# pangsu0613/TransCAR

Hardware: AMD Instinct MI355X
Metric: nuScenes frames/sec (6-cam+radar, 900 queries): fusion decoder (Detr3DHead.forward + box decode), FPN features resident in HBM (higher is better)
Workload: dtype f32 (linear steps and attention core of the batched launches: f16x2 split operands, 3 v_mfma_f32_16x16x32_f16 products, fp32 accumulate; activations of the 32-row tiles held as two f16 planes; 4- / 8-row tiles: f32 MFMA)

## Files before the change

transcar_amd/csrc/chain.hip:

```cpp
#include <stdlib.h>
#include <string.h>

#include <type_traits>

#include "kernels.hpp"
#ifdef TC_CHAIN_STAMPS
__device__ long long g_cam_stamps[4][8];
#define CAM_STAMP(slot)                                                                        \
  do {                                                                                         \
    if (blockIdx.x == 100 && (threadIdx.x & 63) == 0)                                          \
      g_cam_stamps[(threadIdx.x >> 6) & 3][(slot)] = __builtin_amdgcn_s_memtime();             \
  } while (0)
#endif
#include "rowdev.hpp"
#define TC_ONCE_LD(p) ldg4_stream(p)
#ifdef TC_CHAIN_DUMP
__device__ float* g_chain_dump;
__device__ long long g_chain_dump_floats;
#endif

namespace tc {

namespace {

constexpr int CH_NW = 4;
constexpr int CH_NT = CH_NW * 64;
constexpr int CH_NW_MAX = 8;
constexpr int nw_of(int R) { return R == 32 ? 8 : 4; }
constexpr int LD5 = 516;
constexpr int LD2 = 260;
constexpr int LDL = 36;

struct StepRes {
  const float* p0; const float* p1; const float* p2; const float* p3;
  float* gd; float* gt;
  int K, N, gld, gmod;
  short kind, src, src2, dst, res, act, flags, sync, rep, si;
  int src_off, src2_off;
  int pad_;
};
struct EpiRec {
  float* gd; float* gt;
  int dst_off, res_off, dst_ld, res_ld;
  int gld, act, flags, N;
  int has_bias, woff;
  int drop_site;
  int pad1;
};
struct PreRec { const float* first; int nidx; int pad; };
template <int NW> struct StepAllT { StepRes r; EpiRec e; PreRec p[NW]; };
using StepAll = StepAllT<CH_NW>;
static_assert(sizeof(StepAllT<CH_NW>) % 16 == 0 && sizeof(StepAllT<CH_NW_MAX>) % 16 == 0, "records are copied 16 bytes at a time");
template <int N, int NW = CH_NW> struct Recs { StepAllT<NW> s[N]; };

constexpr int HM_WORDS = 8;
static_assert(HM_WORDS * 8 <= LDL * 4 && (LDL * 4) % 8 == 0, "hit masks live in a row of the logit buffer");
template <int R, int NREC>
struct ChainLds {
  StepAllT<nw_of(R)> recs[NREC];
  float unit[4][R][LD2];
  float l[R][LDL];
  float box[R][12];
  float cen[R][4];
  int gate[R];
  int rowg[R];
};
static_assert(LD5 * 1 <= 2 * LD2, "the 512-wide tile must fit two units");

#ifdef TC_CHAIN_STAMPS
#define CHAIN_DBG(v) (v)
#else
#define CHAIN_DBG(v) 0
#endif

#define MFMA44(a, b, c, grp) __builtin_amdgcn_mfma_f32_4x4x1f32((a), (b), (c), 4, (grp), 0)

enum Buf : short { B_NONE = -1, B_A = 0 , B_X , B_U1, B_U2, B_U3, B_L };
enum Kind : short {
  K_END = 0, K_LOAD, K_LINEAR, K_LN, K_POSENC, K_SAMPLE, K_REFUPD, K_TOKENS, K_RADAR_ATTN, K_BOXADD, K_RADAR_GATE,
  K_NARROW,
  K_NOP,
  K_LOADG,
  K_MASKCOPY,
  K_LN_BWD,
  K_ATTN_BWD,
  K_BOXSIG
};
enum NSpecial : short { N_LOGITS = -1, N_CODE = -2, N_CLS = -3 };
// ... 171 lines not shown
enum TSel : short { T_NONE = -1, T_QP = 0, T_AO, T_X1, T_X2, T_H, T_FF, T_X3, T_C0, T_C1, T_C2, T_C3, T_T0, T_T1, T_TREG,
                    E_U0, E_U1, E_U2, E_POS, E_F0, E_F1, E_F2, E_MEM, T_COUNT };
constexpr short RADAR_TAPE[17] = {T_NONE, T_QP, T_AO, T_X1, T_X2, T_H, T_FF, T_X3, T_C0, T_T0, T_C1, T_T1, T_C2, T_C3,
                                  T_TREG, T_NONE, T_NONE};
constexpr short ENC_TAPE[10] = {T_NONE, E_U1, E_F0, E_U2, E_F1, E_F2, E_MEM, T_NONE, T_NONE, T_NONE};
constexpr short ENC_TAPE2[10] = {T_NONE, E_U0, T_NONE, T_NONE, T_NONE, T_NONE, E_POS, T_NONE, T_NONE, T_NONE};
constexpr short BWD_TAPE[19] = {T_NONE, T_T1, T_T0, T_NONE, T_NONE, T_NONE, T_C2, T_NONE, T_C0, T_NONE, T_X2, T_NONE,
                                T_H, T_NONE, T_X1, T_NONE, T_NONE, T_NONE, T_NONE};
constexpr short BWD_TAPE2[19] = {T_NONE, T_NONE, T_NONE, T_NONE, T_NONE, T_NONE, T_C3, T_NONE, T_C1, T_NONE, T_FF, T_NONE,
                                 T_NONE, T_NONE, T_NONE, T_NONE, T_NONE, T_NONE, T_NONE};

constexpr int MAX_PAIRS = 48;
constexpr int RADAR_PAIRS = 14;

struct ChainDev {
  int program, M, Q, code, ncls, nlogits, has_next, nlayers;
  int total, early_n;
  float* g[G_COUNT]; int g_ld[G_COUNT]; int g_mod[G_COUNT];
  float qscale; int qpad;
  DropK drop;
  int dbg;
  int tile_rows;
  int matrix_path;
  int last_cls_only;
  const float* ref_in; int ref_mod; float* ref_out; float* box_m;
  CamK cam; unsigned long long* pair_counter;
  const float* pre; const int* premask;
  const float* tokens; int RI, T, pad_mult;
  const float* ref_last; const float* box_in;
  int cen_from_box;
  float rmin[TC_MAX_RADAR_LAYERS], rmax[TC_MAX_RADAR_LAYERS];
  float* all_box; int* hits;
  const int* row_perm;
  float* tape[T_COUNT]; size_t tape_stride; size_t hits_stride;
  DropK rdrop;
  const float* bwd_cxy[TC_MAX_RADAR_LAYERS]; int bwd_ldc[TC_MAX_RADAR_LAYERS];
  const float* bwd_box[TC_MAX_RADAR_LAYERS];
  int* range_status;
  const float* loss_vals;
  float* loss_out;
  const DetAcc* detp;
};
struct ChainK : ChainDev {
  tc_linear pairs[MAX_PAIRS];
  tc_linear gpairs[MAX_PAIRS];
  float* dy[D_COUNT]; size_t dy_stride = 0;
  const float* d_cls = nullptr; const float* d_box = nullptr;
  float* dkv[TC_MAX_RADAR_LAYERS] = {nullptr, nullptr, nullptr};
  size_t w16_delta = 0;
  int npoints = 1;
  int refine = 1;
  int l0_seq = 0;
};

inline bool generic_xattn(const ChainK& k) { return k.npoints > 1 || k.cam.num_levels < 4; }

constexpr int table_steps(int prog) {
  return (prog == PROG_DECODER ? (int)(sizeof(PROG_DECODER_T) / sizeof(StepDesc))
          : prog == PROG_PROLOGUE ? (int)(sizeof(PROG_PROLOGUE_T) / sizeof(StepDesc))
          : prog_is_enc_full(prog) ? (int)(sizeof(PROG_RADAR_ENC_T) / sizeof(StepDesc))
          : prog == PROG_RADAR_ENC_A ? (int)(sizeof(PROG_RADAR_ENC_A_T) / sizeof(StepDesc))
          : prog == PROG_RADAR_ENC_B ? (int)(sizeof(PROG_RADAR_ENC_B_T) / sizeof(StepDesc))
          : prog == PROG_RADAR_BWD ? (int)(sizeof(PROG_RADAR_BWD_T) / sizeof(StepDesc))
          : prog == PROG_DECODER_HEADS ? (int)(sizeof(PROG_DECODER_HEADS_T) / sizeof(StepDesc))
                                     : (int)(sizeof(PROG_RADAR_LAYER_T) / sizeof(StepDesc))) - 1;
}
// ... 1078 lines not shown
#pragma unroll
        for (int ri = 0; ri < EARLY_RW; ++ri) {
          int grow = min(m0 + wave + ri * NW, M - 1);
          if (mod > 0) grow = grow % mod;
          early_v[j][ri] = TC_ONCE_LD(gsrc + (size_t)grow * ld + 4 * lane);
        }
      }
    }
    START_STAMP(41);
#pragma unroll
    for (int j = 0; j < EARLY_MAX; ++j) {
      if (j < early_n) {
        float* dst = reinterpret_cast<float*>(smem_raw) + recs[j].e.dst_off;
#pragma unroll
        for (int ri = 0; ri < EARLY_RW; ++ri) {
          const int row = wave + ri * NW;
          if (row < R) act_st4<PL>(dst + row * LD2, 4 * lane, early_v[j][ri]);
        }
      }
    }
  }
#pragma unroll
  for (int t = 0; t < REC_TRIPS; ++t) {
    const int i = threadIdx.x + t * NT;
    if (i < REC16) reinterpret_cast<int4*>(&S.recs[0])[i] = rec_v[t];
  }
  START_STAMP(43);

  if (prog_is_radar(PROG)) {
    auto row_of = [&](int row) {
      const int pos = min(m0 + row, M - 1);
      return k.row_perm != nullptr ? k.row_perm[pos] : pos;
    };
    if (threadIdx.x < R) S.rowg[threadIdx.x] = row_of(threadIdx.x);
    for (int row = wave; row < R; row += NW) {
      const int grow = row_of(row);
      act_st4<PL>(&S.unit[0][row][0], 4 * lane, TC_ONCE_LD(k.g[G_QF] + (size_t)grow * 256 + 4 * lane));
    }
    {
      const int row = threadIdx.x >> 4, j = threadIdx.x & 15;
      if (row < R) {
        const int grow = row_of(row);
        if (j < k.code) S.box[row][j] = k.box_in[(size_t)grow * k.code + j];
        if (j >= 12 && j < 15) {
          const int c = j - 12;
          if (k.cen_from_box) {
            S.cen[row][c] = k.box_in[(size_t)grow * k.code + (c == 2 ? 4 : c)];
          } else {
            const float r = k.ref_last[(size_t)grow * 3 + c];
            const float* pc = k.cam.pc;
            S.cen[row][c] = c < 2 ? __fadd_rn(__fmul_rn(r, pc[3 + c] - pc[c]), pc[c]) : r;
          }
        }
      }
    }
  }
  if constexpr (PROG == PROG_RADAR_BWD) {
    for (int i = threadIdx.x; i < R * LD2; i += NT) (&S.unit[0][0][0])[i] = 0.0f;
    if (threadIdx.x < R * 12) (&S.box[0][0])[threadIdx.x] = 0.0f;
    if (threadIdx.x < R) S.gate[threadIdx.x] = 0;
  }
  __syncthreads();

  START_STAMP(46);
#ifdef TC_CHAIN_STAMPS
  int stamp_i = 0;
  STEP_STAMP();
#endif

  auto do_ln = [&](const StepRes& r) {
    constexpr int NR = R / NW;
    const float* a = buf_ptr(S, r.src); const int lda = buf_ld(r.src);
    const float* c = buf_ptr(S, r.src2); const int ldc = buf_ld(r.src2);
    const bool xp = (r.flags & F_LN_XP) != 0;
    const float* dd = xp ? nullptr : buf_ptr(S, r.res);
// ... 51 lines not shown
    s.dst = nullptr; s.dst_ld = 0; s.res = nullptr; s.res_ld = 0; s.gate = nullptr;
    s.act = 0; s.scale = 1.0f; s.scale_cols = 0;
    s.gdst = nullptr; s.gdst_ld = 0; s.gt = nullptr; s.gt_ld = 0; s.gt_rpb = 1;
    s.m0 = m0; s.M = M;
    s.woff = (r.flags & F_WAVE1) ? 1 : 0;
    s.dbg = k.dbg;
    s.sub_on = 0;
    s.drop_site = 0; s.drop_seed = 0; s.drop_thr = 0; s.drop_scale = 1.0f; s.drop_stride = 0; s.drop_q = 0;
    s.rowg = nullptr; s.gpre = 0; s.cmask = nullptr; s.cscale = 1.0f;
    s.dst_pl = 0; s.res_pl = 0; s.range_flag = nullptr;
    return s;
  };
  auto epi_spec = [&](int j) {
    const EpiRec e = load_uniform<EpiRec>(S.recs[j].e);
    float* base = reinterpret_cast<float*>(smem_raw);
    LinSpec s;
    s.K = 0; s.N = e.N; s.W = nullptr;
    s.bias = e.has_bias ? base : nullptr;
    s.src = nullptr; s.src_ld = 0; s.src2 = nullptr; s.src2_ld = 0;
    s.dst = e.dst_off >= 0 ? base + e.dst_off : nullptr; s.dst_ld = e.dst_ld;
    s.res = e.res_off >= 0 ? base + e.res_off : nullptr; s.res_ld = e.res_ld;
    s.gate = (e.flags & F_GATE) ? &S.gate[0] : nullptr;
    s.act = e.act;
    s.scale = (e.flags & F_SCALEQ) ? k.qscale : 1.0f; s.scale_cols = (e.flags & F_SCALEQ) ? 256 : 0;
    s.gdst = e.gd; s.gdst_ld = e.gld;
    s.gt = (e.flags & F_CMASK) ? nullptr : e.gt; s.gt_ld = k.qpad; s.gt_rpb = k.Q;
    s.cmask = (e.flags & F_CMASK) ? e.gt : nullptr;
    s.cscale = (e.flags & F_CMASK_SCALE) ? k.rdrop.scale : 1.0f;
    s.m0 = m0; s.M = M;
    s.woff = e.woff;
    s.dbg = 0;
    s.sub_on = 0;
    s.drop_site = 0; s.drop_seed = 0; s.drop_thr = 0; s.drop_scale = 1.0f; s.drop_stride = 0; s.drop_q = 0;
    s.rowg = (prog_is_radar(PROG) && k.row_perm != nullptr) ? &S.rowg[0] : nullptr;
    s.gpre = (e.flags & F_GPRE) ? 1 : 0;
    s.dst_pl = PL && e.dst_ld != LDL; s.res_pl = PL && e.res_ld != LDL;
    s.range_flag = MM == 1 ? k.range_status : nullptr;
    if (DROP) {
      if constexpr (PROG == PROG_RADAR_TRAIN) {
        s.drop_site = e.drop_site; s.drop_seed = k.rdrop.seed; s.drop_thr = k.rdrop.thr; s.drop_scale = k.rdrop.scale;
      } else {
        s.drop_site = e.drop_site; s.drop_seed = k.drop.seed; s.drop_thr = k.drop.thr; s.drop_scale = k.drop.scale;
        s.drop_stride = k.drop.seed_stride; s.drop_q = (int)k.drop.rows_per_sample;
      }
    }
    return s;
  };

  auto tile_has_hit = [&]() {
    int any = 0;
#pragma unroll
    for (int i = 0; i < R; ++i) any |= S.gate[i];
    return __builtin_amdgcn_readfirstlane(any) > 0;
  };

#ifdef TC_CHAIN_DUMP
  auto dump_step = [&](int step, int dst_id) {
    if constexpr (PROG == PROG_RADAR) {
      __syncthreads();
      float* out = g_chain_dump;
      const float* src = buf_ptr(S, dst_id);
      if (out != nullptr && src != nullptr && dst_id != B_L && (long long)(step + 1) * M * 256 <= g_chain_dump_floats) {
        const int ld = buf_ld(dst_id);
        for (int row = wave; row < R; row += NW)
          if (m0 + row < M)
            st4(out + ((size_t)step * M + S.rowg[row]) * 256 + 4 * lane, *reinterpret_cast<const float4*>(src + row * ld + 4 * lane));
      }
// ... 1146 lines not shown

template <bool MP>
static int launch_dual(const ChainK& kd, const ChainK& ke, int part, hipStream_t s) {
  const int rows = tile_rows(kd);
  const char* what = "chain(decoder + radar_encode)";
#define TC_DUAL(RA, RB, MM, PRE)                                                                      \
  (part == 1 ? launch_dual_r<RA, RB, PROG_RADAR_ENC_A, MM, PRE, MP>(kd, ke, s, what)                  \
   : part == 2 ? launch_dual_r<RA, RB, PROG_RADAR_ENC_B, MM, PRE, MP>(kd, ke, s, what)                \
               : launch_dual_r<RA, RB, PROG_RADAR_ENC, MM, PRE, MP>(kd, ke, s, what))
  if (rows == 4) return TC_DUAL(4, 4, 0, false);
  if (rows == 8) return TC_DUAL(8, 8, 0, false);
  if (rows == 32) {
    TC_REQUIRE(use_f16x2(kd), "%s: 32-row tiles exist on the f16x2 matrix path only", what);
    if (kd.pre != nullptr) return TC_DUAL(32, 32, 1, true);
    return TC_DUAL(32, 32, 1, false);
  }
  if (use_f16x2(kd) && kd.pre != nullptr) return TC_DUAL(16, 16, 1, true);
  if (use_f16x2(kd)) return TC_DUAL(16, 16, 1, false);
  return TC_DUAL(16, 16, 0, false);
#undef TC_DUAL
}

int launch_decoder_chain_with_encoders(const DecoderChainArgs& d, const RadarEncodeArgs& e, int part,
                                       hipStream_t s) {
  ChainK kd, ke;
  int rc = make_decoder_k(d, kd);
  if (rc != 0) return rc;
  rc = make_radar_enc_k(e, ke, part);
  if (rc != 0) return rc;
  TC_REQUIRE(kd.drop.thr == 0, "decoder dropout: launch the encoders on their own (launch_radar_encode)");
  return generic_xattn(kd) ? launch_dual<true>(kd, ke, part, s) : launch_dual<false>(kd, ke, part, s);
}

int launch_radar_chain(const RadarChainArgs& a, hipStream_t s) {
  TC_REQUIRE(a.code <= 10 && a.ncls <= 32, "radar_chain: code=%d ncls=%d", a.code, a.ncls);
  TC_REQUIRE(a.nlayers >= 1 && a.nlayers <= TC_MAX_RADAR_LAYERS, "radar_chain: nlayers=%d", a.nlayers);
  ChainK k;
  init_k(k);
  k.program = PROG_RADAR; k.M = a.M; k.Q = a.Q; k.code = a.code; k.ncls = a.ncls; k.nlayers = a.nlayers;
  k.w16_delta = a.w[0].packed16_delta;
  k.row_perm = a.row_perm;
  k.has_next = 1;
  for (int r = 0; r < a.nlayers; ++r) {
    const tc_radar_layer& w = a.w[r];
    tc_linear* p = &k.pairs[r * RADAR_PAIRS];
    p[0] = w.attn.in_proj; p[1] = w.attn.out_proj; p[2] = tc_linear{w.norm2.g, w.norm2.b};
    p[3] = w.linear1; p[4] = w.linear2; p[5] = tc_linear{w.norm3.g, w.norm3.b};
    p[6] = w.final_cls.l0; p[7] = tc_linear{w.final_cls.n1.g, w.final_cls.n1.b}; p[8] = w.final_cls.l3;
    p[9] = tc_linear{w.final_cls.n4.g, w.final_cls.n4.b}; p[10] = w.final_cls.l6;
    p[11] = w.final_reg.l0; p[12] = w.final_reg.l2; p[13] = w.final_reg.l4;
    k.rmin[r] = w.radius_min; k.rmax[r] = w.radius_max;
    k.g[G_KV0 + r] = const_cast<float*>(a.kv[r]);
  }
  k.g[G_QF] = const_cast<float*>(a.qf);
  k.g[G_CLS] = a.all_cls; k.g_ld[G_CLS] = a.ncls;
  k.qscale = a.qscale;
  k.tokens = a.tokens; k.RI = a.RI; k.T = a.T; k.pad_mult = a.pad_mult;
  k.ref_last = a.ref_last; k.box_in = a.box_m; k.cen_from_box = a.cen_from_box;
  TC_REQUIRE(a.cen_from_box || a.ref_last != nullptr, "radar_chain: ref_last is null");
  for (int i = 0; i < 6; ++i) k.cam.pc[i] = a.pc[i];
  k.all_box = a.all_box; k.hits = a.hits;
  TC_REQUIRE(a.tile_rows == 0 || a.tile_rows == 4 || a.tile_rows == 8 || a.tile_rows == 16 || a.tile_rows == 32,
             "radar_chain: tile_rows=%d (0 = automatic, 4, 8, 16 or 32)", a.tile_rows);
  k.tile_rows = a.tile_rows; k.last_cls_only = a.last_cls_only; k.matrix_path = a.matrix_path;
  k.range_status = a.range_status;
  if (a.tape != nullptr) {
    TC_REQUIRE(a.row_perm == nullptr && !a.last_cls_only, "radar_chain: the training forward takes the rows in their own order");
    k.program = PROG_RADAR_TRAIN;
    for (int i = 0; i < T_COUNT; ++i) k.tape[i] = a.tape[i];
    k.tape_stride = a.tape_stride; k.hits_stride = a.hits_stride; k.rdrop = a.drop;
    if (k.tile_rows >= 16 || (k.tile_rows == 0 && a.M > 2048)) k.tile_rows = 8;
  }
  return launch(k, s, "chain(radar)");
}
// ... 155 lines not shown
```

transcar_amd/csrc/head.hip:

```cpp
#include <math.h>
#include <stdarg.h>
#include <stdlib.h>
#include <string.h>

#include "kernels.hpp"

namespace tc {

static thread_local char g_err[512] = "";

void set_error(const char* fmt, ...) {
  va_list ap;
  va_start(ap, fmt);
  vsnprintf(g_err, sizeof(g_err), fmt, ap);
  va_end(ap);
}

int check_launch(const char* what) {
  hipError_t e = hipGetLastError();
  if (e != hipSuccess) {
    set_error("%s: %s", what, hipGetErrorString(e));
    return (int)e;
  }
  return 0;
// ... 253 lines not shown
      }
    }
    if (radar && !ddrop && lid == enc_first) TC_TRY(launch_decoder_chain_with_encoders(d, re, L > 1 ? 1 : 0, s));
    else if (radar && !ddrop && L > 1 && lid == enc_first + 1) TC_TRY(launch_decoder_chain_with_encoders(d, re, 2, s));
    else TC_TRY(launch_decoder_chain(d, s));
  }
  if (opt.phase == 1) return 0;
  if (!refine)
    TC_TRY(launch_ref_broadcast(folded ? w->l0_init_reference : h.init_ref, folded ? Q : 0, h.inter_refs, rows, L, s));
  if (aux) {
    if (aux->init_reference) {
      if (folded) {
        for (int b = 0; b < B; ++b)
          TC_HIP(hipMemcpyAsync(aux->init_reference + (size_t)b * Q * 3, w->l0_init_reference,
                                (size_t)Q * 3 * 4, hipMemcpyDeviceToDevice, s));
      } else {
        TC_HIP(hipMemcpyAsync(aux->init_reference, h.init_ref, (size_t)rows * 3 * 4, hipMemcpyDeviceToDevice, s));
      }
    }
  }
  if (!radar) return 0;
  RadarChainArgs rc;
  rc.qf = h.hs + (size_t)(L - 1) * rows * C;
  rc.ref_last = h.inter_refs + (size_t)(L - 1) * rows * 3;
  rc.box_m = h.box_m; rc.tokens = radar_tokens; rc.RI = w->radar_in_dims;
  for (int r = 0; r < TC_MAX_RADAR_LAYERS; ++r) { rc.kv[r] = h.kv3[r]; rc.w[r] = w->radar[r]; }
  rc.nlayers = w->num_radar_layers; rc.Q = Q; rc.T = T; rc.pad_mult = pad_mult; rc.code = code;
  rc.ncls = ncls; rc.M = rows; rc.qscale = 1.0f / sqrtf((float)(C / TC_RADAR_HEADS));
  for (int i = 0; i < 6; ++i) rc.pc[i] = w->pc_range[i];
  rc.all_cls = all_cls_scores; rc.all_box = all_bbox_preds; rc.hits = h.hits;
  rc.tile_rows = opt.chain_tile_rows; rc.last_cls_only = opt.last_level_cls_only; rc.matrix_path = opt.matrix_path;
  rc.range_status = opt.range_status;
  if (opt.radar_row_order == 2 || (opt.radar_row_order == 0 && rows > 1024)) {
    TC_TRY(launch_radar_compact(rc.ref_last, rc.box_m, code, 0, w->pc_range, radar_tokens, w->radar_in_dims, B, Q, T,
                                w->radar[0].radius_min, w->radar[0].radius_max, h.hitflag, h.perm, s));
    rc.row_perm = h.perm;
  }
  TC_TRY(launch_radar_chain(rc, s));
  if (aux && aux->radar_hit_counts)
    TC_HIP(hipMemcpyAsync(aux->radar_hit_counts, h.hits, (size_t)w->num_radar_layers * rows * 4,
                          hipMemcpyDeviceToDevice, s));
  return 0;
}

struct PackItem { const float* src; int N, K; const float** slot; bool narrow; bool absent; };

static int collect_pack_items(const tc_head_weights* w, tc_head_weights* v, PackItem* it) {
  const int C = w->embed_dims, F = w->ffn_dims, NL = w->num_cams * w->num_levels * head_points(w);
  const int code = w->code_size, ncls = w->num_classes;
  int n = 0;
  auto add = [&](const tc_linear& src, tc_linear& dst, int N, int K, bool narrow = false, bool absent = false) {
    it[n].src = src.w; it[n].N = N; it[n].K = K; it[n].slot = &dst.w; it[n].narrow = narrow; it[n].absent = absent; ++n;
  };
  add(w->reference_points, v->reference_points, 3, C);
  for (int l = 0; l < w->num_layers; ++l) {
    const tc_decoder_layer& a = w->layers[l]; tc_decoder_layer& b = v->layers[l];
    add(a.self_attn.in_proj, b.self_attn.in_proj, 3 * C, C);
    add(a.self_attn.out_proj, b.self_attn.out_proj, C, C);
    add(a.attention_weights, b.attention_weights, NL, C);
    add(a.output_proj, b.output_proj, C, C);
    add(a.position_encoder.l3, b.position_encoder.l3, C, C);
    add(a.ffn0, b.ffn0, F, C);
    add(a.ffn1, b.ffn1, C, F);
    const bool noreg = a.reg.l0.w == nullptr;
    add(a.reg.l0, b.reg.l0, C, C, false, noreg);
    add(a.reg.l2, b.reg.l2, C, C, false, noreg);
    add(a.reg.l4, b.reg.l4, code, C, true, noreg);
  }
  if (w->num_radar_layers > 0) {
// ... 306 lines not shown
  TC_TRY(read_options(options, opt));
  HeadWs h;
  const size_t need = head_ws_layout(w, B, T, workspace, workspace_bytes, &h);
  TC_REQUIRE(need <= workspace_bytes, "workspace too small: need %zu, have %zu", need, workspace_bytes);
  hipStream_t s = as_stream(stream);
  const int Q = w->num_query, C = w->embed_dims, rows = B * Q, rt = B * T;
  const int code = w->code_size, ncls = w->num_classes;
  RadarEncodeArgs re;
  re.tokens = radar_tokens; re.RI = w->radar_in_dims; re.M = rt;
  re.rpe = w->radar_position_encoder; re.f0 = w->radar_feat0; re.f2 = w->radar_feat2;
  re.f4 = w->radar_feat4; re.nlayers = w->num_radar_layers;
  for (int r = 0; r < TC_MAX_RADAR_LAYERS; ++r) {
    const tc_mha& m = w->radar[r].attn;
    re.kvproj[r] = tc_linear{m.in_proj.w ? m.in_proj.w + (size_t)C * C : nullptr,
                             m.in_proj.b ? m.in_proj.b + C : nullptr};
    re.kv[r] = h.kv3[r];
  }
  re.radar_feat = h.radar_feat;
  re.w16_delta = w->packed16_delta; re.matrix_path = opt.matrix_path;
  if (!opt.reuse_radar_kv) TC_TRY(launch_radar_encode(re, s));
  RadarChainArgs rc;
  rc.qf = hs_last; rc.ref_last = ref_last; rc.box_m = prev_box; rc.tokens = radar_tokens;
  rc.RI = w->radar_in_dims;
  for (int r = 0; r < num_layers; ++r) { rc.kv[r] = h.kv3[first_layer + r]; rc.w[r] = w->radar[first_layer + r]; }
  rc.nlayers = num_layers; rc.Q = Q; rc.T = T; rc.pad_mult = pad_mult; rc.code = code; rc.ncls = ncls;
  rc.M = rows; rc.qscale = 1.0f / sqrtf((float)(C / TC_RADAR_HEADS));
  for (int i = 0; i < 6; ++i) rc.pc[i] = w->pc_range[i];
  rc.all_cls = all_cls_scores + (size_t)first_layer * rows * ncls;
  rc.all_box = all_bbox_preds + (size_t)first_layer * rows * code;
  rc.hits = h.hits; rc.tile_rows = opt.chain_tile_rows; rc.last_cls_only = opt.last_level_cls_only; rc.matrix_path = opt.matrix_path;
  rc.range_status = opt.range_status;
  rc.cen_from_box = first_layer > 0;
  if (opt.radar_row_order == 2 || (opt.radar_row_order == 0 && rows > 1024)) {
    TC_TRY(launch_radar_compact(ref_last, prev_box, code, rc.cen_from_box, w->pc_range, radar_tokens, w->radar_in_dims,
                                B, Q, T, w->radar[first_layer].radius_min, w->radar[first_layer].radius_max,
                                h.hitflag, h.perm, s));
    rc.row_perm = h.perm;
  }
  TC_TRY(launch_radar_chain(rc, s));
  if (hit_counts != nullptr)
    TC_HIP(hipMemcpyAsync(hit_counts + (size_t)first_layer * rows, h.hits, (size_t)num_layers * rows * 4,
                          hipMemcpyDeviceToDevice, s));
  return 0;
}

int tc_radar_gate_selfcheck(int n_radii, unsigned long long seed, unsigned long long* mismatches,
                            tc_stream_t stream) {
  return launch_gate_selfcheck(n_radii, seed, mismatches, as_stream(stream));
}

int tc_rowops_selfcheck(int n_blocks, unsigned long long seed, unsigned long long* mismatches, tc_stream_t stream) {
  return launch_rowops_selfcheck(n_blocks, seed, mismatches, as_stream(stream));
}

size_t tc_box_decode_workspace_bytes(int B, int Q, int num_classes) {
  return box_decode_ws_bytes(B, Q, num_classes);
}

int tc_box_decode_topk(const float* cls_scores, const float* bbox_preds, int B, int Q,
                       int num_classes, int code_size, int max_num, const float* post_center_range,
                       float* boxes, float* scores, int* labels, unsigned char* valid,
                       void* workspace, size_t workspace_bytes, tc_stream_t stream) {
  return launch_box_decode(cls_scores, bbox_preds, B, Q, num_classes, code_size, max_num,
                           post_center_range, boxes, scores, labels, valid, workspace,
                           workspace_bytes, as_stream(stream));
}

int tc_box_decode_kept(const float* cls_scores, const float* bbox_preds, int B, int Q, int num_classes, int code_size,
                       int max_num, const float* post_center_range, float score_threshold, int use_threshold,
                       int z_shift, float* kept_boxes, float* kept_scores, long long* kept_labels, int* kept_count,
// ... 513 lines not shown
```

transcar_amd/csrc/kernels.hpp:

```cpp
#pragma once
#include "common.hpp"
#include "../../include/transcar_hip.h"

namespace tc {

struct GemmArgs {
  const float* X = nullptr;  int ldx = 0;
  const float* X2 = nullptr; int x2_cols = 0;
  const float* W = nullptr;  int ldw = 0;
  const float* bias = nullptr;
  const float* R = nullptr;  int ldr = 0;
  const int* rowgate = nullptr;
  float* Y = nullptr;        int ldy = 0;
  float* Yt = nullptr;
  int t_col0 = 0, t_ld = 0, t_rows_per_batch = 1;
  int M = 0, K = 0, N = 0;
  int act = 0;
  float scale = 1.0f; int scale_cols = 0;
};
int launch_gemm(const GemmArgs& a, hipStream_t s);

struct LnArgs {
  const float* a = nullptr;
  const float* b = nullptr;
// ... 68 lines not shown
int launch_decoder_chain(const DecoderChainArgs& a, hipStream_t s);
constexpr int TC_L0_VARIANTS = 5;
size_t decoder_l0_const_floats(int Q);
int decoder_l0_variant(int M, int tile_rows, int matrix_path);
int launch_decoder_l0_consts(const DecoderChainArgs& a, int variant, float* consts, hipStream_t s);

struct RadarEncodeArgs {
  const float* tokens; int RI, M;
  tc_pos_encoder rpe; tc_linear f0, f2, f4;
  int nlayers; tc_linear kvproj[TC_MAX_RADAR_LAYERS]; float* kv[TC_MAX_RADAR_LAYERS];
  float* radar_feat;
  size_t w16_delta = 0;
  float* const* tape = nullptr;
  int matrix_path = 0;
  int* range_status = nullptr;
};
int launch_radar_encode(const RadarEncodeArgs& a, hipStream_t s);
int launch_decoder_chain_with_encoders(const DecoderChainArgs& d, const RadarEncodeArgs& e, int part,
                                       hipStream_t s);

struct RadarChainArgs {
  const float* qf; const float* ref_last; const float* box_m;
  const float* tokens; int RI;
  const float* kv[TC_MAX_RADAR_LAYERS];
  tc_radar_layer w[TC_MAX_RADAR_LAYERS];
  int nlayers, Q, T, pad_mult, code, ncls, M;
  float qscale; float pc[6];
  float* all_cls; float* all_box; int* hits;
  int tile_rows = 0;
  int matrix_path = 0;
  int last_cls_only = 0;
  int cen_from_box = 0;
  const int* row_perm = nullptr;
  float* const* tape = nullptr; size_t tape_stride = 0, hits_stride = 0;
  DropK drop = DropK{0, 0, 1.0f, 0, 1500, 0, 0, 0};
  int* range_status = nullptr;
};
enum DySlot { DY_DBOX = 0, DY_DT1, DY_DT0, DY_DC2, DY_DC0, DY_DFF, DY_DH, DY_DPROJ, DY_DQP, DY_DCLS, DY_COUNT };
struct RadarBwdChainArgs {
  tc_radar_layer wT[TC_MAX_RADAR_LAYERS];
  tc_radar_layer w[TC_MAX_RADAR_LAYERS];
  tc_radar_layer grads[TC_MAX_RADAR_LAYERS];
  const float* kv[TC_MAX_RADAR_LAYERS]; float* dkv[TC_MAX_RADAR_LAYERS];
  const float* cxy[TC_MAX_RADAR_LAYERS]; int ld_c[TC_MAX_RADAR_LAYERS]; const float* box[TC_MAX_RADAR_LAYERS];
  float* const* tape; size_t tape_stride, hits_stride; const int* hits;
  float* const* dy; size_t dy_stride;
  const float* d_cls; const float* d_box;
  const float* loss_vals = nullptr;
  float* loss_out = nullptr;
  const float* tokens; int RI, T, pad_mult;
  int nlayers, Q, M, code, ncls;
  float qscale;
  DropK drop;
  int tile_rows = 0;
  const DetAcc* det_device = nullptr;
};
int launch_radar_chain_bwd(const RadarBwdChainArgs& a, hipStream_t s);
enum TapeSlot { TS_QP = 0, TS_AO, TS_X1, TS_X2, TS_H, TS_SUM, TS_X3, TS_C0, TS_C1, TS_C2, TS_C3, TS_T0, TS_T1, TS_TREG,
                TS_U0, TS_U1, TS_U2, TS_POS, TS_F0, TS_F1, TS_F2, TS_MEM, TS_COUNT };
int launch_radar_chain(const RadarChainArgs& a, hipStream_t s);

struct DecoderHeadsArgs {
  int levels, M;
  tc_cls_branch cls[TC_MAX_LAYERS]; tc_reg_branch reg[TC_MAX_LAYERS];
  size_t w16_delta = 0;
  const float* hs;
  const float* init_ref;
  const float* inter_refs;
  float* all_cls; float* all_box;
  int ncls, code; float pc[6];
  int tile_rows = 0, matrix_path = 0;
  int* range_status = nullptr;
};
int launch_decoder_heads(const DecoderHeadsArgs& a, hipStream_t s);

int launch_radar_compact(const float* ref_last, const float* box, int code, int cen_from_box,
                         const float* pc6_host, const float* tokens, int RI, int B, int Q, int T,
                         float rmin, float rmax, int* flags, int* perm, hipStream_t s);

int launch_gate_selfcheck(int n_radii, unsigned long long seed, unsigned long long* mismatches, hipStream_t s);
int launch_rowops_selfcheck(int n_blocks, unsigned long long seed, unsigned long long* mismatches, hipStream_t s);

inline bool heads_ok(int num_heads) { return num_heads == 4 || num_heads == 8 || num_heads == 16; }
int launch_self_attn_core(const float* q, const float* k, int ld, const float* vt, int ldt,
                          float* out, int ldo, int B, int Q, int H, int D, hipStream_t s,
                          const DropK* drop = nullptr);
struct PreGatherArgs {
  CamSampleArgs cam; int M, ref_mod; float* out; int* mask;
};
int launch_self_attn_core_x(const float* q, const float* k, int ld, const float* vt, int ldt, float* out, int ldo,
                            int B, int Q, int H, int D, hipStream_t s, const DropK* drop = nullptr,
                            const PreGatherArgs* pregather = nullptr);

// ... 76 lines not shown
```

transcar_amd/csrc/radar_compact.hip:

```cpp
#include "kernels.hpp"
#include "rowdev.hpp"

namespace tc {

struct CompactK {
  const float* ref_last; const float* box; const float* tokens;
  int code, cen_from_box, RI, B, Q, T;
  float pc[6]; float rmin, rmax;
  int* flags;
};

__global__ __launch_bounds__(256) void radar_hit_flags_kernel(CompactK p) {
  __shared__ float sx[256], sy[256];
  const int lane = threadIdx.x & 63, wave = threadIdx.x >> 6;
  const int tiles = (p.Q + 15) / 16;
  const int b = blockIdx.x / tiles, q0 = (blockIdx.x - b * tiles) * 16;
  float cx[4], cy[4], b3[4], b6[4], b7[4];
  bool any[4];
#pragma unroll
  for (int i = 0; i < 4; ++i) {
    const int q = min(q0 + 4 * wave + i, p.Q - 1);
    const size_t row = (size_t)b * p.Q + q;
    const float* bx = p.box + row * p.code;
    if (p.cen_from_box) { cx[i] = bx[0]; cy[i] = bx[1]; }
// ... 70 lines not shown
  unsigned long long h = (seed + 0x9E3779B97F4A7C15ull * (unsigned long long)(r + 1));
  h ^= h >> 30; h *= 0xBF58476D1CE4E5B9ull; h ^= h >> 27; h *= 0x94D049BB133111EBull; h ^= h >> 31;
  float rad = 0.5f + 1.5f * (float)(h >> 40) * (1.0f / 16777216.0f);
  if (r == 0) rad = 0.5f;
  if (r == 1) rad = 1.0f;
  if (r == 2) rad = 2.0f;
  const float tstar = sqrt_threshold(rad);
  const unsigned centre = __builtin_bit_cast(unsigned, rad * rad);
  unsigned long long bad = 0;
  for (int i = threadIdx.x; i < 512 + 4096; i += 256) {
    float t;
    if (i < 512) t = __builtin_bit_cast(float, centre - 256u + (unsigned)i);
    else {
      unsigned long long g = h + 0xD1B54A32D192ED03ull * (unsigned long long)i;
      g ^= g >> 29; g *= 0xBF58476D1CE4E5B9ull; g ^= g >> 32;
      t = -1.0f + 10.0f * (float)(g >> 40) * (1.0f / 16777216.0f);
    }
    const bool ref = sqrtf(fmaxf(t, 1e-30f)) < rad;
    const bool fast = fmaxf(t, 1e-30f) < tstar;
    bad += ref != fast;
  }
  if (bad) atomicAdd(mismatches, bad);
}

int launch_gate_selfcheck(int n_radii, unsigned long long seed, unsigned long long* mismatches, hipStream_t s) {
  TC_REQUIRE(n_radii > 0 && mismatches != nullptr, "radar_gate_selfcheck: bad arguments");
  hipLaunchKernelGGL(gate_selfcheck_kernel, dim3(n_radii), dim3(256), 0, s, n_radii, seed, mismatches);
  return check_launch("radar_gate_selfcheck");
}

int launch_radar_compact(const float* ref_last, const float* box, int code, int cen_from_box,
                         const float* pc6_host, const float* tokens, int RI, int B, int Q, int T,
                         float rmin, float rmax, int* flags, int* perm, hipStream_t s) {
  TC_REQUIRE(B > 0 && Q > 0 && T > 0 && flags != nullptr && perm != nullptr, "radar_compact: bad arguments");
  CompactK p;
  p.ref_last = ref_last; p.box = box; p.tokens = tokens; p.code = code; p.cen_from_box = cen_from_box;
  p.RI = RI; p.B = B; p.Q = Q; p.T = T; p.rmin = rmin; p.rmax = rmax; p.flags = flags;
  for (int i = 0; i < 6; ++i) p.pc[i] = pc6_host[i];
  hipLaunchKernelGGL(radar_hit_flags_kernel, dim3(B * ((Q + 15) / 16)), dim3(256), 0, s, p);
  hipLaunchKernelGGL(radar_partition_kernel, dim3(B), dim3(256), 0, s, flags, Q, perm);
  return check_launch("radar_compact");
}

}
```

transcar_amd/csrc/rowdev.hpp:

```cpp
#pragma once
#include "common.hpp"
#include "../../include/transcar_hip.h"

namespace tc {

__device__ __forceinline__ float4 relu4(float4 v) {
  return make_float4(relu_(v.x), relu_(v.y), relu_(v.z), relu_(v.w));
}
__device__ __forceinline__ float4 add4(float4 a, float4 b) {
  return make_float4(a.x + b.x, a.y + b.y, a.z + b.z, a.w + b.w);
}

__device__ __forceinline__ float4 ln_row(float4 v, const float* g, const float* b, int lane) {
  const float4 gg = ld4(g + 4 * lane), bb = ld4(b + 4 * lane);
  float s = wave_sum(v.x + v.y + v.z + v.w);
  const float mean = s * (1.0f / 256.0f);
  float4 d = make_float4(v.x - mean, v.y - mean, v.z - mean, v.w - mean);
  float q = wave_sum(d.x * d.x + d.y * d.y + d.z * d.z + d.w * d.w);
  const float rstd = 1.0f / sqrtf(q * (1.0f / 256.0f) + 1e-5f);
  return make_float4(d.x * rstd * gg.x + bb.x, d.y * rstd * gg.y + bb.y,
                     d.z * rstd * gg.z + bb.z, d.w * rstd * gg.w + bb.w);
}

__device__ __forceinline__ float wave_sum4_packed(float a, float b, float c, float d) {
  float t;
  asm volatile(
      "s_nop 1\n\t"
      "v_add_f32_dpp %0, %0, %0 quad_perm:[1,0,3,2] row_mask:0xf bank_mask:0xf\n\t"
      "v_add_f32_dpp %1, %1, %1 quad_perm:[1,0,3,2] row_mask:0xf bank_mask:0xf\n\t"
      "v_add_f32_dpp %2, %2, %2 quad_perm:[1,0,3,2] row_mask:0xf bank_mask:0xf\n\t"
      "v_add_f32_dpp %3, %3, %3 quad_perm:[1,0,3,2] row_mask:0xf bank_mask:0xf\n\t"
      "v_add_f32_dpp %0, %0, %0 quad_perm:[2,3,0,1] row_mask:0xf bank_mask:0xf\n\t"
      "v_add_f32_dpp %1, %1, %1 quad_perm:[2,3,0,1] row_mask:0xf bank_mask:0xf\n\t"
      "v_add_f32_dpp %2, %2, %2 quad_perm:[2,3,0,1] row_mask:0xf bank_mask:0xf\n\t"
      "v_add_f32_dpp %3, %3, %3 quad_perm:[2,3,0,1] row_mask:0xf bank_mask:0xf\n\t"
// ... 546 lines not shown
```

Baseline: 10420.

## Fuse radar row partition into radar chain kernel via per-tile ranking

Drops the separate radar_partition_kernel launch when the 32-row inference radar chain runs. Each chain tile now reads the hit flags for its one or two samples, ranks hits before misses using wave ballots and popcounts, and fills its own row index table in LDS. This removes one kernel launch and a global permutation round-trip. In exchange every tile redoes the ranking over up to Q flags and adds two block barriers before its loads.

```diff
diff --git a/transcar_amd/csrc/chain.hip b/transcar_amd/csrc/chain.hip
--- a/transcar_amd/csrc/chain.hip
+++ b/transcar_amd/csrc/chain.hip
@@ -54,6 +54,7 @@
 template <int N, int NW = CH_NW> struct Recs { StepAllT<NW> s[N]; };
 
 constexpr int HM_WORDS = 8;
+constexpr int RANK_CH = 2;
 static_assert(HM_WORDS * 8 <= LDL * 4 && (LDL * 4) % 8 == 0, "hit masks live in a row of the logit buffer");
 template <int R, int NREC>
 struct ChainLds {
@@ -291,6 +292,7 @@
   float rmin[TC_MAX_RADAR_LAYERS], rmax[TC_MAX_RADAR_LAYERS];
   float* all_box; int* hits;
   const int* row_perm;
+  const int* row_flags;
   float* tape[T_COUNT]; size_t tape_stride; size_t hits_stride;
   DropK rdrop;
   const float* bwd_cxy[TC_MAX_RADAR_LAYERS]; int bwd_ldc[TC_MAX_RADAR_LAYERS];
@@ -1435,15 +1437,75 @@
       const int pos = min(m0 + row, M - 1);
       return k.row_perm != nullptr ? k.row_perm[pos] : pos;
     };
-    if (threadIdx.x < R) S.rowg[threadIdx.x] = row_of(threadIdx.x);
+    const bool own_rank = R == 32 && PROG == PROG_RADAR && k.row_flags != nullptr;
+    if constexpr (R == 32 && PROG == PROG_RADAR) {
+      if (own_rank) {
+        const int Q = k.Q, pos_end = min(m0 + R, M);
+        const int bA = m0 / Q, nb = (pos_end - 1) / Q - bA + 1;
+        int* ws = &S.gate[0];
+        static_assert(2 * RANK_CH * NW <= R, "the rank scratch lives in S.gate");
+        bool in[RANK_CH], v[2][RANK_CH];
+        unsigned long long mh[2][RANK_CH];
+#pragma unroll
+        for (int sm = 0; sm < 2; ++sm) {
+          const int* f = k.row_flags + (size_t)(bA + min(sm, nb - 1)) * Q;
+#pragma unroll
+          for (int c = 0; c < RANK_CH; ++c) {
+            const int i = c * NT + (int)threadIdx.x;
+            in[c] = i < Q;
+            v[sm][c] = f[min(i, Q - 1)] != 0;
+          }
+        }
+#pragma unroll
+        for (int sm = 0; sm < 2; ++sm) {
+#pragma unroll
+          for (int c = 0; c < RANK_CH; ++c) {
+            mh[sm][c] = __ballot(in[c] && v[sm][c]);
+            if (lane == 0) ws[(sm * RANK_CH + c) * NW + wave] = __popcll(mh[sm][c]);
+          }
+        }
+        __syncthreads();
+#pragma unroll
+        for (int sm = 0; sm < 2; ++sm) {
+          if (sm < nb) {
+            const int b = bA + sm;
+            RankBase rb[RANK_CH];
+            int hit_base = 0, miss_base = 0;
+#pragma unroll
+            for (int c = 0; c < RANK_CH; ++c) {
+              rb[c] = rank_base(ws + (sm * RANK_CH + c) * NW, NW, wave, min(max(Q - c * NT, 0), NT));
+              miss_base += rb[c].hits_total;
+            }
+#pragma unroll
+            for (int c = 0; c < RANK_CH; ++c) {
+              const int i = c * NT + (int)threadIdx.x;
+              const unsigned long long mm = __ballot(in[c] && !v[sm][c]);
+              if (in[c]) {
+                const unsigned long long below = (1ull << lane) - 1ull;
+                const int pos = b * Q + (v[sm][c] ? hit_base + rb[c].hits_before + __popcll(mh[sm][c] & below)
+                                                  : miss_base + rb[c].misses_before + __popcll(mm & below));
+                if (pos >= m0 && pos < pos_end) {
+                  S.rowg[pos - m0] = b * Q + i;
+                  if (pos == M - 1)
+                    for (int j = pos - m0 + 1; j < R; ++j) S.rowg[j] = b * Q + i;
+                }
+              }
+              hit_base += rb[c].hits_total; miss_base += rb[c].misses_total;
+            }
+          }
+        }
+        __syncthreads();
+      }
+    }
+    if (!own_rank && threadIdx.x < R) S.rowg[threadIdx.x] = row_of(threadIdx.x);
     for (int row = wave; row < R; row += NW) {
-      const int grow = row_of(row);
+      const int grow = own_rank ? S.rowg[row] : row_of(row);
       act_st4<PL>(&S.unit[0][row][0], 4 * lane, TC_ONCE_LD(k.g[G_QF] + (size_t)grow * 256 + 4 * lane));
     }
     {
       const int row = threadIdx.x >> 4, j = threadIdx.x & 15;
       if (row < R) {
-        const int grow = row_of(row);
+        const int grow = own_rank ? S.rowg[row] : row_of(row);
         if (j < k.code) S.box[row][j] = k.box_in[(size_t)grow * k.code + j];
         if (j >= 12 && j < 15) {
           const int c = j - 12;
@@ -1561,7 +1623,7 @@
     s.dbg = 0;
     s.sub_on = 0;
     s.drop_site = 0; s.drop_seed = 0; s.drop_thr = 0; s.drop_scale = 1.0f; s.drop_stride = 0; s.drop_q = 0;
-    s.rowg = (prog_is_radar(PROG) && k.row_perm != nullptr) ? &S.rowg[0] : nullptr;
+    s.rowg = (prog_is_radar(PROG) && (k.row_perm != nullptr || k.row_flags != nullptr)) ? &S.rowg[0] : nullptr;
     s.gpre = (e.flags & F_GPRE) ? 1 : 0;
     s.dst_pl = PL && e.dst_ld != LDL; s.res_pl = PL && e.res_ld != LDL;
     s.range_flag = MM == 1 ? k.range_status : nullptr;
@@ -2774,6 +2836,14 @@
   return generic_xattn(kd) ? launch_dual<true>(kd, ke, part, s) : launch_dual<false>(kd, ke, part, s);
 }
 
+bool radar_chain_ranks_rows(const RadarChainArgs& a) {
+  if (a.tape != nullptr) return false;
+  ChainK k;
+  init_k(k);
+  k.M = a.M; k.tile_rows = a.tile_rows; k.matrix_path = a.matrix_path;
+  return tile_rows(k) == 32 && a.Q >= 32 && a.Q <= RANK_CH * nw_of(32) * 64;
+}
+
 int launch_radar_chain(const RadarChainArgs& a, hipStream_t s) {
   TC_REQUIRE(a.code <= 10 && a.ncls <= 32, "radar_chain: code=%d ncls=%d", a.code, a.ncls);
   TC_REQUIRE(a.nlayers >= 1 && a.nlayers <= TC_MAX_RADAR_LAYERS, "radar_chain: nlayers=%d", a.nlayers);
@@ -2781,7 +2851,9 @@
   init_k(k);
   k.program = PROG_RADAR; k.M = a.M; k.Q = a.Q; k.code = a.code; k.ncls = a.ncls; k.nlayers = a.nlayers;
   k.w16_delta = a.w[0].packed16_delta;
-  k.row_perm = a.row_perm;
+  k.row_perm = a.row_perm; k.row_flags = a.row_flags;
+  TC_REQUIRE(a.row_flags == nullptr || (a.row_perm == nullptr && radar_chain_ranks_rows(a)),
+             "radar_chain: row_flags go with the 32-row inference kernel, and without a row_perm");
   k.has_next = 1;
   for (int r = 0; r < a.nlayers; ++r) {
     const tc_radar_layer& w = a.w[r];
diff --git a/transcar_amd/csrc/head.hip b/transcar_amd/csrc/head.hip
--- a/transcar_amd/csrc/head.hip
+++ b/transcar_amd/csrc/head.hip
@@ -309,9 +309,10 @@
   rc.tile_rows = opt.chain_tile_rows; rc.last_cls_only = opt.last_level_cls_only; rc.matrix_path = opt.matrix_path;
   rc.range_status = opt.range_status;
   if (opt.radar_row_order == 2 || (opt.radar_row_order == 0 && rows > 1024)) {
+    const bool ranks = radar_chain_ranks_rows(rc);
     TC_TRY(launch_radar_compact(rc.ref_last, rc.box_m, code, 0, w->pc_range, radar_tokens, w->radar_in_dims, B, Q, T,
-                                w->radar[0].radius_min, w->radar[0].radius_max, h.hitflag, h.perm, s));
-    rc.row_perm = h.perm;
+                                w->radar[0].radius_min, w->radar[0].radius_max, h.hitflag, ranks ? nullptr : h.perm, s));
+    if (ranks) rc.row_flags = h.hitflag; else rc.row_perm = h.perm;
   }
   TC_TRY(launch_radar_chain(rc, s));
   if (aux && aux->radar_hit_counts)
@@ -684,10 +685,11 @@
   rc.range_status = opt.range_status;
   rc.cen_from_box = first_layer > 0;
   if (opt.radar_row_order == 2 || (opt.radar_row_order == 0 && rows > 1024)) {
+    const bool ranks = radar_chain_ranks_rows(rc);
     TC_TRY(launch_radar_compact(ref_last, prev_box, code, rc.cen_from_box, w->pc_range, radar_tokens, w->radar_in_dims,
                                 B, Q, T, w->radar[first_layer].radius_min, w->radar[first_layer].radius_max,
-                                h.hitflag, h.perm, s));
-    rc.row_perm = h.perm;
+                                h.hitflag, ranks ? nullptr : h.perm, s));
+    if (ranks) rc.row_flags = h.hitflag; else rc.row_perm = h.perm;
   }
   TC_TRY(launch_radar_chain(rc, s));
   if (hit_counts != nullptr)
diff --git a/transcar_amd/csrc/kernels.hpp b/transcar_amd/csrc/kernels.hpp
--- a/transcar_amd/csrc/kernels.hpp
+++ b/transcar_amd/csrc/kernels.hpp
@@ -124,6 +124,7 @@
   int last_cls_only = 0;
   int cen_from_box = 0;
   const int* row_perm = nullptr;
+  const int* row_flags = nullptr;
   float* const* tape = nullptr; size_t tape_stride = 0, hits_stride = 0;
   DropK drop = DropK{0, 0, 1.0f, 0, 1500, 0, 0, 0};
   int* range_status = nullptr;
@@ -151,6 +152,7 @@
 enum TapeSlot { TS_QP = 0, TS_AO, TS_X1, TS_X2, TS_H, TS_SUM, TS_X3, TS_C0, TS_C1, TS_C2, TS_C3, TS_T0, TS_T1, TS_TREG,
                 TS_U0, TS_U1, TS_U2, TS_POS, TS_F0, TS_F1, TS_F2, TS_MEM, TS_COUNT };
 int launch_radar_chain(const RadarChainArgs& a, hipStream_t s);
+bool radar_chain_ranks_rows(const RadarChainArgs& a);
 
 struct DecoderHeadsArgs {
   int levels, M;
diff --git a/transcar_amd/csrc/radar_compact.hip b/transcar_amd/csrc/radar_compact.hip
--- a/transcar_amd/csrc/radar_compact.hip
+++ b/transcar_amd/csrc/radar_compact.hip
@@ -126,13 +126,13 @@
 int launch_radar_compact(const float* ref_last, const float* box, int code, int cen_from_box,
                          const float* pc6_host, const float* tokens, int RI, int B, int Q, int T,
                          float rmin, float rmax, int* flags, int* perm, hipStream_t s) {
-  TC_REQUIRE(B > 0 && Q > 0 && T > 0 && flags != nullptr && perm != nullptr, "radar_compact: bad arguments");
+  TC_REQUIRE(B > 0 && Q > 0 && T > 0 && flags != nullptr, "radar_compact: bad arguments");
   CompactK p;
   p.ref_last = ref_last; p.box = box; p.tokens = tokens; p.code = code; p.cen_from_box = cen_from_box;
   p.RI = RI; p.B = B; p.Q = Q; p.T = T; p.rmin = rmin; p.rmax = rmax; p.flags = flags;
   for (int i = 0; i < 6; ++i) p.pc[i] = pc6_host[i];
   hipLaunchKernelGGL(radar_hit_flags_kernel, dim3(B * ((Q + 15) / 16)), dim3(256), 0, s, p);
-  hipLaunchKernelGGL(radar_partition_kernel, dim3(B), dim3(256), 0, s, flags, Q, perm);
+  if (perm != nullptr) hipLaunchKernelGGL(radar_partition_kernel, dim3(B), dim3(256), 0, s, flags, Q, perm);
   return check_launch("radar_compact");
 }
 
diff --git a/transcar_amd/csrc/rank_rule.hpp b/transcar_amd/csrc/rank_rule.hpp
--- /dev/null
+++ b/transcar_amd/csrc/rank_rule.hpp
@@ -0,0 +1,25 @@
+#pragma once
+
+#if defined(__HIPCC__) || defined(__CUDACC__)
+#define TC_RANK_HD __host__ __device__ __forceinline__
+#else
+#define TC_RANK_HD inline
+#endif
+
+namespace tc {
+
+struct RankBase { int hits_before, misses_before, hits_total, misses_total; };
+
+TC_RANK_HD RankBase rank_base(const int* wave_hits, int nw, int wave, int in_chunk) {
+  RankBase r{0, 0, 0, 0};
+  for (int w = 0; w < nw; ++w) {
+    if (w < wave) r.hits_before += wave_hits[w];
+    r.hits_total += wave_hits[w];
+  }
+  const int rows_before = 64 * wave < in_chunk ? 64 * wave : in_chunk;
+  r.misses_before = rows_before - r.hits_before;
+  r.misses_total = in_chunk - r.hits_total;
+  return r;
+}
+
+}
diff --git a/transcar_amd/csrc/rowdev.hpp b/transcar_amd/csrc/rowdev.hpp
--- a/transcar_amd/csrc/rowdev.hpp
+++ b/transcar_amd/csrc/rowdev.hpp
@@ -1,6 +1,7 @@
 #pragma once
 #include "common.hpp"
 #include "../../include/transcar_hip.h"
+#include "rank_rule.hpp"
 
 namespace tc {
 
```

Result: slower. 10310 (-1.0%).
